# libshoal/Green-Marl

Measured on AMD Instinct MI355X. Metric: edges/s (GTEPS) per PageRank iter, RMAT-26, higher is better.
Workload: dtype f32; 1 GPU; pagerank RMAT-26 (V=67108864, E=1073741824), reference RMAT generator seed 1997 permute=1, d=0.85, fixed iterations; partition=1-D vertex, 1 rank(s), exchange=none, exchange_bytes_per_rank_and_step=0, exchange_packed=False, step_form=single rank, options=15

## Files before the change

### green-marl_amd/csrc/gmx_internal.h

```cpp
#ifndef GMX_INTERNAL_H_
#define GMX_INTERNAL_H_

#include <hip/hip_runtime.h>
#include <stdint.h>
#include <stdio.h>
#include <stdarg.h>
#include <string.h>
#include <time.h>
#include <stdlib.h>
#include <string>
#include <vector>

#include "gmx.h"

void gmx_set_error(const char* fmt, ...);

#define GMX_HIP(call)                                                                      \
    do {                                                                                   \
        hipError_t _e = (call);                                                            \
        if (_e != hipSuccess) {                                                            \
            gmx_set_error("%s:%d: %s -> %s", __FILE__, __LINE__, #call, hipGetErrorString(_e)); \
            return GMX_ERR_HIP;                                                            \
        }                                                                                  \
    } while (0)

#define GMX_CHECK(call)                 \
    do {                                \
        int _s = (call);                \
        if (_s != GMX_OK) return _s;    \
    } while (0)

#define GMX_REQUIRE(cond, ...)          \
    do {                                \
        if (!(cond)) {                  \
            gmx_set_error(__VA_ARGS__); \
            return GMX_ERR_ARG;         \
        }                               \
    } while (0)

template <typename T>
struct dbuf {
    T* p = nullptr;
    size_t n = 0;
    dbuf() {}
    dbuf(const dbuf&) = delete;
    dbuf& operator=(const dbuf&) = delete;
    ~dbuf() { release(); }
    int alloc(size_t count) {
        release();
        n = count;
        size_t bytes = (count ? count : 1) * sizeof(T);
        hipError_t e = hipMalloc((void**) &p, bytes);
        if (e != hipSuccess) {
            p = nullptr;
            n = 0;
            gmx_set_error("hipMalloc(%zu bytes) failed: %s", bytes, hipGetErrorString(e));
            return GMX_ERR_NOMEM;
        }
        return GMX_OK;
    }
    void release() {
        if (p) (void) hipFree(p);
        p = nullptr;
        n = 0;
    }
    T* take() { T* q = p; p = nullptr; n = 0; return q; }
};

struct gmx_event {
    hipEvent_t e = nullptr;
    gmx_event() {}
    gmx_event(gmx_event&& o) : e(o.e) { o.e = nullptr; }
    gmx_event(const gmx_event&) = delete;
    gmx_event& operator=(const gmx_event&) = delete;
    ~gmx_event() { if (e) (void) hipEventDestroy(e); }
    int create() { GMX_HIP(hipEventCreate(&e)); return GMX_OK; }
    operator hipEvent_t() const { return e; }
};
template <typename T>
struct gmx_pinned {
    T* p = nullptr;
    gmx_pinned() {}
    gmx_pinned(const gmx_pinned&) = delete;
    gmx_pinned& operator=(const gmx_pinned&) = delete;
    ~gmx_pinned() { if (p) (void) hipHostFree(p); }
    int alloc(size_t count = 1) {
        if (hipHostMalloc((void**) &p, count * sizeof(T), hipHostMallocDefault) != hipSuccess) {
            p = nullptr;
            gmx_set_error("pinned host allocation (%zu bytes) failed", count * sizeof(T));
            return GMX_ERR_HIP;
        }
        return GMX_OK;
    }
};
template <typename T>
static inline int gmx_read_back(gmx_pinned<T>& host, const T* dev, size_t count = 1) {
    GMX_HIP(hipMemcpyAsync(host.p, dev, count * sizeof(T), hipMemcpyDeviceToHost, 0));
    GMX_HIP(hipStreamSynchronize(0));
    return GMX_OK;
}

static inline int64_t gmx_env_int(const char* name, int64_t dflt, int64_t lo, int64_t hi) {
    const char* e = getenv(name);
    if (!e || !*e) return dflt;
    const long long v = atoll(e);
    return v < lo ? lo : (v > hi ? hi : (int64_t) v);
}

struct gmx_ws_mark { size_t chunk, off; };
void* gmx_ws_alloc(size_t bytes);
gmx_ws_mark gmx_ws_top();
void gmx_ws_rewind(gmx_ws_mark m);
struct gmx_ws_scope {
    gmx_ws_mark m;
    gmx_ws_scope() : m(gmx_ws_top()) {}
    ~gmx_ws_scope() { (void) hipDeviceSynchronize(); gmx_ws_rewind(m); }
    gmx_ws_scope(const gmx_ws_scope&) = delete;
    gmx_ws_scope& operator=(const gmx_ws_scope&) = delete;
};
template <typename T>
struct wbuf {
    T* p = nullptr;
    size_t n = 0;
    wbuf() {}
    wbuf(const wbuf&) = delete;
    wbuf& operator=(const wbuf&) = delete;
    int alloc(size_t count) {
        n = count;
        p = (T*) gmx_ws_alloc((count ? count : 1) * sizeof(T));
        if (!p) { n = 0; return GMX_ERR_NOMEM; }
        return GMX_OK;
    }
    void release() { p = nullptr; n = 0; }
};

struct gmx_bfs;
struct tcd_plan;
void gmx_tcd_plan_free(tcd_plan* p);
struct vc_plan;
void gmx_vc_plan_free(vc_plan* p);
struct spf_scratch;
void gmx_spf_scratch_free(spf_scratch* s);

struct gmx_graph {
    int64_t V = 0, E = 0;
    bool has_reverse = false;
    dbuf<int32_t> begin, node_idx, r_begin, r_node_idx;
    dbuf<int32_t> e_idx2idx;
    bool rows_sorted = true, r_rows_sorted = true;
    int device = 0;
    gmx_pr* pr_cache[4] = {nullptr, nullptr, nullptr, nullptr};
    struct gmx_pr_multi* pr_multi_cache[2] = {nullptr, nullptr};
    bool pr_multi_refused = false;
    int tc_sym_state = -1;
    gmx_graph* tc_oriented = nullptr;
    dbuf<uint32_t> tc_hub_bits;
    int64_t tc_hubs = 0;
    tcd_plan* tcd_cache = nullptr;
    vc_plan* vc_cache = nullptr;
    spf_scratch* spf_cache = nullptr;
    gmx_bfs* bfs_cache = nullptr;
    dbuf<int32_t> bfs_hint;
    dbuf<int32_t> bfs_hub_id;
    int64_t bfs_hubs = 0;
    bool bfs_hint_plain = false;
    gmx_graph* scc_transpose = nullptr;
};

int gmx_bfs_reach(gmx_graph* g, int32_t root, const int32_t** dist, int64_t* edges);
int gmx_bc_seeds(gmx_graph* g, const gmx_node_t* seeds, int32_t nseeds, int skip_root, float* bc_dev, bool zero_bc, hipEvent_t started, int64_t* reached);

int gmx_csr_from_keys(uint64_t* keys, uint64_t* keys_alt, int64_t V, int64_t E,
                      int32_t* begin, int32_t* idx, hipStream_t stream, int32_t* slots = nullptr);
int gmx_keys_from_csr(const int32_t* begin, const int32_t* idx, int64_t V, int64_t E,
                      bool transpose, const int32_t* perm, uint64_t* keys, hipStream_t stream);
int gmx_keys_from_edges(const int32_t* src, const int32_t* dst, int64_t E, bool transpose,
                        const int32_t* perm, uint64_t* keys, hipStream_t stream);
__global__ void iota_kernel(int32_t* __restrict__ a, int64_t n);

struct pr_cold;
struct pr_cold_params {
    int elem;
    int nranks;
    int64_t slice;
    int64_t T;
    int64_t row_lo;
    int64_t nactive;
    const int32_t* index_of_row;
    const int32_t* deg_by_id;
};
int pr_cold_create(const uint64_t* keys, int64_t Ec, const pr_cold_params& prm, hipStream_t s, pr_cold** out);
void pr_cold_free(pr_cold* c);
struct pr_cold_fuse {
    const int32_t* active;
    const int32_t* outdeg_c;
    void* rk_c;
    void* next_owned;
    double base, d;
};
int pr_cold_launch(pr_cold* c, const void* contrib, const pr_cold_fuse* fuse, hipStream_t s);
int pr_cold_set_parts(pr_cold* c, int nparts, const int64_t* act_bound, int64_t hub, int64_t live);
int pr_cold_parts(const pr_cold* c);
int64_t pr_cold_class_items(const pr_cold* c, int cls);
int pr_cold_gather(pr_cold* c, const void* contrib, int cls, hipStream_t s);
int pr_cold_accumulate(pr_cold* c, const pr_cold_fuse* fuse, int part, hipStream_t s);
const double* pr_cold_diff_partials(const pr_cold* c, int64_t* n);
bool pr_cold_covers_all_rows(const pr_cold* c);
bool pr_cold_limb_guard(const pr_cold* c, double d, double N);
const void* pr_cold_partial(const pr_cold* c);
int64_t pr_cold_edges(const pr_cold* c);
int64_t pr_cold_items(const pr_cold* c);

struct gmx_pr_multi;
int gmx_pr_multi_ranks(const gmx_graph* g);
int gmx_pr_multi_create(gmx_graph* g, int elem, int nranks, gmx_pr_multi** out);
int gmx_pr_multi_run(gmx_pr_multi* m, double e, double d, int32_t max_iter, void* rank_host, gmx_stats_t* stats);
void gmx_pr_multi_free(gmx_pr_multi* m);
bool gmx_pr_multi_verified(const gmx_pr_multi* m);

struct gmx_tick {
    bool on;
    double t0;
    const char* who;
    static double now() { struct timespec ts; clock_gettime(CLOCK_MONOTONIC, &ts); return ts.tv_sec + 1e-9 * ts.tv_nsec; }
    explicit gmx_tick(const char* w) : on(getenv("GMX_PLAN_TIMING") != nullptr), t0(0), who(w) { if (on) { (void) hipDeviceSynchronize(); t0 = now(); } }
    void mark(const char* what) {
        if (!on) return;
        (void) hipDeviceSynchronize();
        const double t = now();
        fprintf(stderr, "gmx timing %s: %-28s %8.2f ms\n", who, what, (t - t0) * 1e3);
        t0 = t;
    }
};

void gmx_touch_pagerank();
void gmx_touch_pr_cold();
void gmx_touch_bfs();
void gmx_touch_sssp();
void gmx_touch_nbrcount();
void gmx_touch_scc();
void gmx_touch_comm();
void gmx_touch_pf();
void gmx_touch_bc_batch();
void gmx_touch_tcd();
void gmx_touch_vcover();
void gmx_touch_match();
void gmx_touch_spf();
void gmx_touch_route();
void gmx_touch_walk();
void gmx_touch_wcc();
void gmx_touch_kcore();
void gmx_touch_msf();
void gmx_warm_modules();

static inline int gmx_bits_for(int64_t v) {
    int b = 1;
    while ((1LL << b) < v && b < 32) b++;
    return b;
}

#endif
```

### green-marl_amd/csrc/gmx_pr_cold.hip

```cpp
#pragma clang fp contract(off)

#include "gmx_internal.h"

#include <algorithm>
#include <rocprim/rocprim.hpp>

#define PRC_G 32
#define PRC_BLK_GROUPS 16
#define PRC_LDS_BYTES 131072
#define PRC_STAGE_BYTES 2048
#define PRC_LDS_LIMIT 163840
static constexpr int prc_tile_elems(int elem) { return (PRC_LDS_LIMIT - 16 * (PRC_STAGE_BYTES + 64 * elem) - 64) / elem; }
static constexpr int prc_tile_elems_classed(int elem) {
    return (PRC_LDS_LIMIT - 16 * 64 * elem - 64) / elem < 32768 ? (PRC_LDS_LIMIT - 16 * 64 * elem - 64) / elem / 8 * 8 : 32768;
}
#define PRC_THREADS 1024
#define PRC_WAVES (PRC_THREADS / 64)
#define PRC_UNROLL 4
#define PRC_PAD 0xffffu
#define PRC_END 0x8000u
#define PRC_Q1P 0
#define PRC_Q1E 64
#define PRC_Q2 128

// ... 564 lines not shown
#undef PRC_PROCESS
}

typedef float prc_f32x2 __attribute__((ext_vector_type(2)));
typedef double prc_f64x2 __attribute__((ext_vector_type(2)));

template <typename S, int FORM> struct prc_form_stores {
    static constexpr int NP = FORM == PRC_FORM_H ? 1 : 8 >> (FORM - PRC_FORM_E1);
    static constexpr int value = (NP * (int) sizeof(S) + 15) / 16;
};

template <typename S, int NP> __device__ __forceinline__ void prc_store_results(S* __restrict__ dst, const S (&out)[NP]);
template <> __device__ __forceinline__ void prc_store_results<float, 1>(float* __restrict__ dst, const float (&out)[1]) { __builtin_nontemporal_store(out[0], dst); }
template <> __device__ __forceinline__ void prc_store_results<float, 2>(float* __restrict__ dst, const float (&out)[2]) {
    prc_f32x2 v; v.x = out[0]; v.y = out[1];
    __builtin_nontemporal_store(v, (prc_f32x2*) dst);
}
template <> __device__ __forceinline__ void prc_store_results<float, 4>(float* __restrict__ dst, const float (&out)[4]) {
    prc_f32x4 v; v.x = out[0]; v.y = out[1]; v.z = out[2]; v.w = out[3];
    __builtin_nontemporal_store(v, (prc_f32x4*) dst);
}
template <> __device__ __forceinline__ void prc_store_results<float, 8>(float* __restrict__ dst, const float (&out)[8]) {
    prc_f32x4 a, b; a.x = out[0]; a.y = out[1]; a.z = out[2]; a.w = out[3]; b.x = out[4]; b.y = out[5]; b.z = out[6]; b.w = out[7];
    __builtin_nontemporal_store(a, (prc_f32x4*) dst);
    __builtin_nontemporal_store(b, (prc_f32x4*) dst + 1);
}
template <> __device__ __forceinline__ void prc_store_results<double, 1>(double* __restrict__ dst, const double (&out)[1]) { __builtin_nontemporal_store(out[0], dst); }
template <> __device__ __forceinline__ void prc_store_results<double, 2>(double* __restrict__ dst, const double (&out)[2]) {
    prc_f64x2 v; v.x = out[0]; v.y = out[1];
    __builtin_nontemporal_store(v, (prc_f64x2*) dst);
}
template <> __device__ __forceinline__ void prc_store_results<double, 4>(double* __restrict__ dst, const double (&out)[4]) {
#pragma unroll
    for (int q = 0; q < 2; q++) { prc_f64x2 v; v.x = out[2 * q]; v.y = out[2 * q + 1]; __builtin_nontemporal_store(v, (prc_f64x2*) dst + q); }
}
template <> __device__ __forceinline__ void prc_store_results<double, 8>(double* __restrict__ dst, const double (&out)[8]) {
#pragma unroll
    for (int q = 0; q < 4; q++) { prc_f64x2 v; v.x = out[2 * q]; v.y = out[2 * q + 1]; __builtin_nontemporal_store(v, (prc_f64x2*) dst + q); }
}

template <typename S, int L>
__device__ __forceinline__ void prc_block_E(const S* __restrict__ s_tile, const prc_u32x4 cur, const int32_t o, S* __restrict__ val, const int lane) {
    constexpr int NP = 8 / L;
    constexpr int K = (NP * (int) sizeof(S) + 15) / 16;
    const unsigned w[4] = {cur.x, cur.y, cur.z, cur.w};
    S fv[8];
#pragma unroll
    for (int u = 0; u < 8; u++) fv[u] = s_tile[__builtin_amdgcn_ubfe(w[u >> 1], 16 * (u & 1), 15)];
    S out[NP];
#pragma unroll
    for (int q = 0; q < NP; q++) {
        if (L == 1) out[q] = fv[q];
        else {
            double acc = (double) fv[q * L];
#pragma unroll
            for (int j = 1; j < L; j++) acc += (double) fv[q * L + j];
            out[q] = (S) acc;
        }
    }
    if constexpr (K == 1) {
        PRC_CHECK(o >= 0 && (o & (NP - 1)) == 0);
        prc_store_results<S, NP>(val + (o + (lane & 3) * NP), out);
    } else {
        constexpr int R = 16 / (int) sizeof(S), CPG = K / 2;
        const int o_lo = __builtin_amdgcn_update_dpp(0, o, 0x114, 0xf, 0xf, true);
        const int o_hi = __builtin_amdgcn_update_dpp(0, o, 0x104, 0xf, 0xf, true);
        const bool upper = (lane & 4) != 0;
        const int o_even = upper ? o_lo : o, o_odd = upper ? o : o_hi;
        const int m = lane & 7;
#pragma unroll
        for (int q = 0; q < K; q++) {
            S piece[R];
#pragma unroll
            for (int r = 0; r < R; r++) piece[r] = out[q * R + r];
            const int at = (q / CPG ? o_odd : o_even) + (q % CPG) * 8 * R + R * m;
            PRC_CHECK(at >= 0 && (at & (R - 1)) == 0);
            prc_store_results<S, R>(val + at, piece);
        }
    }
}

template <typename S>
__device__ __forceinline__ void prc_block_H(const S* __restrict__ s_tile, S* __restrict__ stage, const prc_u32x4 cur, const int32_t o,
                                            S* __restrict__ val, const unsigned sink, const int lane) {
    const unsigned w[4] = {cur.x, cur.y, cur.z, cur.w};
    S fv[8];
#pragma unroll
    for (int u = 0; u < 8; u++) fv[u] = s_tile[__builtin_amdgcn_ubfe(w[u >> 1], 16 * (u & 1), 15)];
    double v = (double) fv[0];
#pragma unroll
    for (int u = 1; u < 8; u++) v += (double) fv[u];
    const int endm = __builtin_amdgcn_sbfe((int) w[3], 31, 1);
    int f = prc_dpp_i<PRC_DPP_WAVE_SHR1, 0xf>(endm) & 1;
    prc_seg_step<PRC_DPP_ROW_SHR(1), 0xf>(v, f);
    prc_seg_step<PRC_DPP_ROW_SHR(2), 0xf>(v, f);
    prc_seg_step<PRC_DPP_ROW_SHR(4), 0xf>(v, f);
    prc_seg_step<PRC_DPP_ROW_SHR(8), 0xf>(v, f);
    prc_seg_step<PRC_DPP_BCAST15, 0xa>(v, f);
    prc_seg_step<PRC_DPP_BCAST31, 0xc>(v, f);
    const unsigned long long ends = __ballot(endm != 0);
    const int total = __builtin_popcountll(ends);
    const int ord = (int) __builtin_amdgcn_mbcnt_hi((unsigned) (ends >> 32), __builtin_amdgcn_mbcnt_lo((unsigned) ends, 0u));
    const unsigned g4 = (unsigned) (ends >> (lane & ~3)) & 0xfu;
    const int gbase = ord - __builtin_popcount(g4 & ((1u << (lane & 3)) - 1u));
    const int shift = o - gbase;
    const unsigned long long live = __ballot(g4 != 0u);
    const int shift0 = __builtin_amdgcn_readlane(shift, live ? __builtin_ctzll(live) : 0);
    const bool one_run = __ballot(g4 != 0u && shift != shift0) == 0ull;
    const S x = (S) v;
    unsigned at;
    S y;
    if (one_run) {
        if (endm) stage[ord] = x;
        __builtin_amdgcn_wave_barrier();
        __builtin_amdgcn_s_waitcnt(0xc07f);
        __builtin_amdgcn_wave_barrier();
        y = stage[lane];
        at = lane < total ? (unsigned) (shift0 + lane) : sink;
        __builtin_amdgcn_wave_barrier();
    } else {
        y = x;
        at = endm ? (unsigned) (shift + ord) : sink;
    }
    PRC_CHECK(at <= sink);
    val[at] = y;
}

template <typename S, int FORM>
__device__ __forceinline__ void prc_class_block(const S* __restrict__ s_tile, S* __restrict__ stage, const prc_u32x4 cur, const int32_t o,
                                                S* __restrict__ val, const unsigned sink, const int lane) {
    if constexpr (FORM == PRC_FORM_H) prc_block_H<S>(s_tile, stage, cur, o, val, sink, lane);
    else prc_block_E<S, 1 << (FORM - PRC_FORM_E1)>(s_tile, cur, o, val, lane);
}

#define PRC_SET_WAIT_N(t, N)                                                                                        \
    asm volatile("s_waitcnt vmcnt(%8)"                                                                              \
                 : "+v"((t).e0), "+v"((t).e1), "+v"((t).e2), "+v"((t).e3), "+v"((t).o0), "+v"((t).o1), "+v"((t).o2), "+v"((t).o3) \
                 : "n"(N) : "memory")

template <typename S, int FORM>
__device__ __forceinline__ void prc_class_item(const prc_item1 d, const S* __restrict__ s_tile, S* __restrict__ stage,
                                               const uint16_t* __restrict__ srcl, const int32_t* __restrict__ ob,
                                               S* __restrict__ val, const unsigned sink, const int wv, const int lane) {
    constexpr int NST = prc_form_stores<S, FORM>::value;
    const int nblocks = (d.g1 - d.g0) / PRC_BLK_GROUPS;
    const int nsuper = nblocks / (PRC_WAVES * PRC_PAIR_DEPTH);
    const prc_u32x4* in = (const prc_u32x4*) srcl + ((int64_t) d.g0 * (PRC_G / 8) + wv * 64 + lane);
    const int32_t* obp = ob + (d.g0 + wv * PRC_BLK_GROUPS + (lane >> 2));
    constexpr int64_t IN_STEP = PRC_PAIR_DEPTH * PRC_WAVES * 64;
    constexpr int64_t OB_STEP = PRC_PAIR_DEPTH * PRC_WAVES * PRC_BLK_GROUPS;
    if (nsuper > 0) {
        prc_set A, B;
#define PRC_PROCESS(t)                                                                  \
    do {                                                                                \
        prc_class_block<S, FORM>(s_tile, stage, (t).e0, (t).o0, val, sink, lane);       \
        prc_class_block<S, FORM>(s_tile, stage, (t).e1, (t).o1, val, sink, lane);       \
        prc_class_block<S, FORM>(s_tile, stage, (t).e2, (t).o2, val, sink, lane);       \
        prc_class_block<S, FORM>(s_tile, stage, (t).e3, (t).o3, val, sink, lane);       \
    } while (0)
        prc_set_load(A, in, obp);
        {
            const int kn = 1 < nsuper ? 1 : 0;
            prc_set_load(B, in + kn * IN_STEP, obp + kn * OB_STEP);
        }
        PRC_SET_WAIT_N(A, 8);
        PRC_PROCESS(A);
        int k = 1;
#pragma unroll 1
        for (; k + 1 < nsuper; k += 2) {
            prc_set_load(A, in + (int64_t) (k + 1) * IN_STEP, obp + (int64_t) (k + 1) * OB_STEP);
            PRC_SET_WAIT_N(B, 4 * NST + 8);
            PRC_PROCESS(B);
            const int kn = k + 2 < nsuper ? k + 2 : k + 1;
            prc_set_load(B, in + (int64_t) kn * IN_STEP, obp + (int64_t) kn * OB_STEP);
            PRC_SET_WAIT_N(A, 4 * NST + 8);
            PRC_PROCESS(A);
        }
        PRC_SET_WAIT_N(B, 4 * NST);
        if (k < nsuper) PRC_PROCESS(B);
#undef PRC_PROCESS
    }
    {
        const int b0 = nsuper * (PRC_WAVES * PRC_PAIR_DEPTH);
        prc_u32x4 cur[PRC_PAIR_DEPTH];
        int32_t o[PRC_PAIR_DEPTH];
#pragma unroll
        for (int j = 0; j < PRC_PAIR_DEPTH; j++)
            if (b0 + j * PRC_WAVES + wv < nblocks) {
                const int64_t off = (int64_t) (b0 + j * PRC_WAVES);
                cur[j] = __builtin_nontemporal_load(in + off * 64);
                o[j] = __builtin_nontemporal_load(obp + off * PRC_BLK_GROUPS);
            }
#pragma unroll
        for (int j = 0; j < PRC_PAIR_DEPTH; j++)
            if (b0 + j * PRC_WAVES + wv < nblocks) prc_class_block<S, FORM>(s_tile, stage, cur[j], o[j], val, sink, lane);
    }
}

template <typename S>
__device__ __forceinline__ void prc_edge_item(const prc_item1 d, const S* __restrict__ s_tile,
                                              const uint16_t* __restrict__ srcl, const int32_t* __restrict__ ob,
                                              S* __restrict__ val, const int wv, const int lane) {
    typedef typename prc_vec4<S>::type V4;
    const int npieces = (d.g1 - d.g0 + 7) >> 3;
    for (int base = 0; base < npieces; base += PRC_WAVES * PRC_UNROLL) {
        prc_u32x2 ids[PRC_UNROLL];
        int32_t o[PRC_UNROLL];
#pragma unroll
        for (int u = 0; u < PRC_UNROLL; u++) {
            const int pc = base + u * PRC_WAVES + wv;
            const int g = d.g0 + pc * 8 + (lane >> 3);
            o[u] = -1;
            if (pc < npieces && g < d.g1) {
                ids[u] = __builtin_nontemporal_load((const prc_u32x2*) srcl + (int64_t) g * (PRC_G / 4) + (lane & 7));
                o[u] = __builtin_nontemporal_load(ob + g);
            }
        }
#pragma unroll
        for (int u = 0; u < PRC_UNROLL; u++) {
            if (o[u] < 0) continue;
            V4 v;
            v.x = s_tile[ids[u].x & 0x7fffu];
            v.y = s_tile[(ids[u].x >> 16) & 0x7fffu];
            v.z = s_tile[ids[u].y & 0x7fffu];
            v.w = s_tile[(ids[u].y >> 16) & 0x7fffu];
            __builtin_nontemporal_store(v, (V4*) (val + o[u]) + (lane & 7));
        }
    }
}

template <typename S, int TILE, bool CLASSED>
__global__ void __launch_bounds__(PRC_THREADS)
pr_cold_tile_kernel(const prc_item1* __restrict__ items, int n_items, unsigned int* __restrict__ queue,
                    const S* __restrict__ contrib, const int32_t* __restrict__ org, int nranks, int64_t span, int64_t slice, int64_t T,
                    const uint16_t* __restrict__ srcl, const int32_t* __restrict__ ob, S* __restrict__ val, unsigned sink_base,
                    unsigned qbase, const int32_t* __restrict__ vst) {
    __shared__ S s_tile[TILE];
    __shared__ S s_stage[PRC_WAVES][CLASSED ? 64 : PRC_STAGE_BYTES / sizeof(S) + 64];
    __shared__ int s_item;
    const int tid = threadIdx.x, lane = tid & 63;
    const int wv = __builtin_amdgcn_readfirstlane(tid >> 6);
    const unsigned sink = sink_base + (blockIdx.x * PRC_WAVES + wv) * 64 + lane;
    int loaded = -1;
    for (;;) {
        __syncthreads();
        if (tid == 0) s_item = (int) (atomicAdd(&queue[CLASSED ? PRC_Q1E : PRC_Q1P], 1u) - qbase);
        __syncthreads();
        const int it = s_item;
        if ((unsigned) it >= (unsigned) n_items) break;
        const prc_item1 d = items[it];
        if (d.tile != loaded) {
            prc_load_tile<S, TILE>(s_tile, d.tile, org, contrib, nranks, span, slice, T);
            loaded = d.tile;
            __syncthreads();
        }
        if constexpr (CLASSED) {
            const int32_t* vs = vst + ((int64_t) d.tile << PRC_CLS_BITS);
            for (int cls = PRC_CL_E1; cls <= PRC_CL_H; cls++) {
                const int32_t lo = max(d.g0, vs[cls]), hi = min(d.g1, vs[cls + 1]);
                if (lo >= hi) continue;
                const prc_item1 seg{d.tile, lo, hi, cls + 1};
                switch (cls) {
                case PRC_CL_E1: prc_class_item<S, PRC_FORM_E1>(seg, s_tile, s_stage[wv], srcl, ob, val, sink, wv, lane); break;
                case PRC_CL_E2: prc_class_item<S, PRC_FORM_E2>(seg, s_tile, s_stage[wv], srcl, ob, val, sink, wv, lane); break;
                case PRC_CL_E4: prc_class_item<S, PRC_FORM_E4>(seg, s_tile, s_stage[wv], srcl, ob, val, sink, wv, lane); break;
                case PRC_CL_E8: prc_class_item<S, PRC_FORM_E8>(seg, s_tile, s_stage[wv], srcl, ob, val, sink, wv, lane); break;
                default: prc_class_item<S, PRC_FORM_H>(seg, s_tile, s_stage[wv], srcl, ob, val, sink, wv, lane); break;
                }
            }
        } else {
            if (d.form == PRC_FORM_PAIR) prc_pair_item<S>(d, s_tile, s_stage[wv], srcl, ob, val, sink, wv, lane);
            else prc_edge_item<S>(d, s_tile, srcl, ob, val, wv, lane);
        }
    }
}

__device__ __forceinline__ unsigned long long prc_fix_hi(double v) { return (unsigned long long) (long long) (v * 0x1p62); }

template <typename S>
__device__ __forceinline__ void prc_finish_row(const pr_cold_fuse& fz, int64_t i, double sum, double& diff_acc) {
    const int32_t od = __builtin_nontemporal_load(fz.outdeg_c + i);
    const int64_t r = __builtin_nontemporal_load(fz.active + i);
    const double old = (double) __builtin_nontemporal_load((const S*) fz.rk_c + i);
    const S vs = (S) (fz.base + fz.d * sum);
    diff_acc += fabs((double) vs - old);
    __builtin_nontemporal_store(vs, (S*) fz.rk_c + i);
    __builtin_nontemporal_store(od > 0 ? (S) ((double) vs / (double) od) : (S) 0, (S*) fz.next_owned + r);
}

template <int THREADS>
__device__ __forceinline__ void prc_block_diff(double diff_acc, double* s_red, double* __restrict__ dst) {
#pragma unroll
    for (int off = 32; off > 0; off >>= 1) diff_acc += __shfl_down(diff_acc, off, 64);
    if ((threadIdx.x & 63) == 0) s_red[threadIdx.x >> 6] = diff_acc;
    __syncthreads();
    if (threadIdx.x == 0) {
        double t = 0.0;
#pragma unroll
        for (int w = 0; w < THREADS / 64; w++) t += s_red[w];
        *dst = t;
    }
}

template <typename S, int BINROWS, int LIMBS, bool FUSE>
__global__ void __launch_bounds__(PRC_THREADS)
pr_cold_accum_kernel(const prc_item2* __restrict__ items, int n_items, unsigned int* __restrict__ queue,
                     const uint16_t* __restrict__ rowl, const S* __restrict__ val, int64_t nactive, double lo_scale,
                     S* __restrict__ cold, unsigned long long* __restrict__ scratch, pr_cold_fuse fz,
                     double* __restrict__ diff_part, unsigned qbase) {
    typedef typename prc_vec4<S>::type V4;
    __shared__ unsigned long long s_acc[LIMBS * BINROWS];
    __shared__ double s_red[PRC_WAVES];
    __shared__ int s_item;
    const int tid = threadIdx.x, lane = tid & 63;
    const int wv = __builtin_amdgcn_readfirstlane(tid >> 6);
    for (;;) {
        __syncthreads();
        if (tid == 0) s_item = (int) (atomicAdd(&queue[PRC_Q2], 1u) - qbase);
#pragma unroll 4
        for (int i = tid; i < LIMBS * BINROWS; i += PRC_THREADS) s_acc[i] = 0ull;
        __syncthreads();
        const int it = s_item;
        if ((unsigned) it >= (unsigned) n_items) break;
        const prc_item2 d = items[it];
        const int npieces = (d.g1 - d.g0 + 7) >> 3;
        for (int base = 0; base < npieces; base += PRC_WAVES * PRC_UNROLL) {
            prc_u32x2 ids[PRC_UNROLL];
            V4 v[PRC_UNROLL];
            bool ok[PRC_UNROLL];
#pragma unroll
            for (int u = 0; u < PRC_UNROLL; u++) {
                const int pc = base + u * PRC_WAVES + wv;
                const int g = d.g0 + pc * 8 + (lane >> 3);
                ok[u] = pc < npieces && g < d.g1;
                if (ok[u]) {
                    const int64_t at = (int64_t) g * (PRC_G / 4) + (lane & 7);
                    ids[u] = __builtin_nontemporal_load((const prc_u32x2*) rowl + at);
                    v[u] = __builtin_nontemporal_load((const V4*) val + at);
                }
            }
#pragma unroll
            for (int u = 0; u < PRC_UNROLL; u++) {
                if (!ok[u]) continue;
                const unsigned r[4] = {ids[u].x & 0xffffu, ids[u].x >> 16, ids[u].y & 0xffffu, ids[u].y >> 16};
                const double x[4] = {(double) v[u].x, (double) v[u].y, (double) v[u].z, (double) v[u].w};
#pragma unroll
                for (int j = 0; j < 4; j++) {
                    if (r[j] == PRC_PAD) continue;
                    PRC_CHECK(r[j] < (unsigned) BINROWS && x[j] >= 0.0 && x[j] <= 1.0);
                    const unsigned long long hi = prc_fix_hi(x[j]);
                    __hip_atomic_fetch_add(&s_acc[r[j]], hi, __ATOMIC_RELAXED, __HIP_MEMORY_SCOPE_WORKGROUP);
                    if (LIMBS > 1) {
                        const double rem = x[j] - (double) (long long) hi * 0x1p-62;
                        const unsigned long long lo = (unsigned long long) (long long) (rem * 0x1p62 * lo_scale);
                        __hip_atomic_fetch_add(&s_acc[BINROWS + r[j]], lo, __ATOMIC_RELAXED, __HIP_MEMORY_SCOPE_WORKGROUP);
                    }
                }
            }
        }
        __syncthreads();
        double diff_acc = 0.0;
        if (d.slot < 0) {
            const int64_t i0 = (int64_t) d.bin * BINROWS;
#pragma unroll 4
            for (int r = tid; r < BINROWS; r += PRC_THREADS) {
                if (i0 + r >= nactive) break;
                double sum = (double) (long long) s_acc[r] * 0x1p-62;
                if (LIMBS > 1) sum += (double) (long long) s_acc[BINROWS + r] * (0x1p-62 / lo_scale);
                if (FUSE) prc_finish_row<S>(fz, i0 + r, sum, diff_acc);
                else __builtin_nontemporal_store((S) sum, cold + i0 + r);
            }
        } else {
            unsigned long long* dst = scratch + (int64_t) d.slot * (LIMBS * BINROWS);
#pragma unroll 4
            for (int i = tid; i < LIMBS * BINROWS; i += PRC_THREADS) dst[i] = s_acc[i];
        }
        if (FUSE) prc_block_diff<PRC_THREADS>(diff_acc, s_red, diff_part + it);
    }
}

template <typename S, int BINROWS, int LIMBS, bool FUSE>
__global__ void __launch_bounds__(1024)
pr_cold_reduce_kernel(const prc_item3* __restrict__ items, int64_t nactive, double lo_scale,
                      const unsigned long long* __restrict__ scratch, S* __restrict__ cold, pr_cold_fuse fz,
                      double* __restrict__ diff_part) {
    __shared__ unsigned long long s_part[LIMBS][16][64];
    const prc_item3 d = items[blockIdx.y];
    const int lane = threadIdx.x & 63, wv = threadIdx.x >> 6;
    const int r = blockIdx.x * 64 + lane;
    const int64_t i0 = (int64_t) d.bin * BINROWS;
    unsigned long long hi = 0, lo = 0;
    const unsigned long long* src = scratch + (int64_t) d.slot0 * (LIMBS * BINROWS) + r;
#pragma unroll 4
    for (int s = wv; s < d.nslots; s += 16) {
        hi += __builtin_nontemporal_load(src + (int64_t) s * (LIMBS * BINROWS));
        if (LIMBS > 1) lo += __builtin_nontemporal_load(src + (int64_t) s * (LIMBS * BINROWS) + BINROWS);
    }
    s_part[0][wv][lane] = hi;
    if (LIMBS > 1) s_part[LIMBS - 1][wv][lane] = lo;
    __syncthreads();
    if (wv == 0 && i0 + r < nactive) {
        hi = 0;
        lo = 0;
#pragma unroll
        for (int w = 0; w < 16; w++) {
            hi += s_part[0][w][lane];
            if (LIMBS > 1) lo += s_part[LIMBS - 1][w][lane];
        }
        double v = (double) (long long) hi * 0x1p-62;
        if (LIMBS > 1) v += (double) (long long) lo * (0x1p-62 / lo_scale);
        if (FUSE) {
            double diff_acc = 0.0;
            prc_finish_row<S>(fz, i0 + r, v, diff_acc);
            s_part[0][0][lane] = (unsigned long long) __double_as_longlong(diff_acc);
        } else cold[i0 + r] = (S) v;
    } else if (FUSE && wv == 0) s_part[0][0][lane] = 0ull;
    if (FUSE && wv == 0) {
        __builtin_amdgcn_wave_barrier();
        __builtin_amdgcn_s_waitcnt(0xc07f);
        __builtin_amdgcn_wave_barrier();
        if (lane == 0) {
            double t = 0.0;
            for (int l = 0; l < 64; l++) t += __longlong_as_double((long long) s_part[0][0][l]);
            diff_part[(int64_t) blockIdx.y * gridDim.x + blockIdx.x] = t;
        }
    }
}

#define PRC_FEW_SLOTS 8
template <typename S, int BINROWS, int LIMBS, bool FUSE>
__global__ void __launch_bounds__(256)
pr_cold_reduce_few_kernel(const prc_item3* __restrict__ items, int64_t nactive, double lo_scale,
                          const unsigned long long* __restrict__ scratch, S* __restrict__ cold, pr_cold_fuse fz,
                          double* __restrict__ diff_part) {
    const prc_item3 d = items[blockIdx.y];
    const int lane = threadIdx.x & 63;
    const int rg = blockIdx.x * 4 + (threadIdx.x >> 6);
    const int r = rg * 64 + lane;
    const int64_t i0 = (int64_t) d.bin * BINROWS;
    unsigned long long hi = 0, lo = 0;
    const unsigned long long* src = scratch + (int64_t) d.slot0 * (LIMBS * BINROWS) + r;
#pragma unroll 4
    for (int s = 0; s < d.nslots; s++) {
        hi += __builtin_nontemporal_load(src + (int64_t) s * (LIMBS * BINROWS));
        if (LIMBS > 1) lo += __builtin_nontemporal_load(src + (int64_t) s * (LIMBS * BINROWS) + BINROWS);
    }
    double diff_acc = 0.0;
    if (i0 + r < nactive) {
        double v = (double) (long long) hi * 0x1p-62;
        if (LIMBS > 1) v += (double) (long long) lo * (0x1p-62 / lo_scale);
        if (FUSE) prc_finish_row<S>(fz, i0 + r, v, diff_acc);
        else cold[i0 + r] = (S) v;
    }
    if (FUSE) {
        double t = 0.0;
        for (int l = 0; l < 64; l++) t += __shfl(diff_acc, l, 64);
        if (lane == 0) diff_part[(int64_t) blockIdx.y * (BINROWS / 64) + rg] = t;
    }
}

static int prc_upload_lists(pr_cold* c, const std::vector<uint8_t>* tile_class, const std::vector<int32_t>* bin_part, int nparts) {
    auto by_size1 = [](const prc_item1& a, const prc_item1& b) { return a.g1 - a.g0 > b.g1 - b.g0; };
    auto by_size2 = [](const prc_item2& a, const prc_item2& b) { return a.g1 - a.g0 > b.g1 - b.g0; };
    std::vector<prc_item1> l1;
    for (int k = 0; k < 2; k++) {
        c->o1[k] = (int64_t) l1.size();
        for (int part = 0; part < 3; part++) {
            if (part == 1) c->o1g[k] = (int64_t) l1.size();
            std::vector<prc_item1> a;
            for (const prc_item1& it : (part < 2 ? c->h1p : c->h1e))
                if ((tile_class ? (int) (*tile_class)[(size_t) it.tile] : 0) == k && (part == 2 || (part == 0) == (it.form >= PRC_FORM_E1))) a.push_back(it);
            std::stable_sort(a.begin(), a.end(), by_size1);
            l1.insert(l1.end(), a.begin(), a.end());
        }
    }
    c->o1[2] = (int64_t) l1.size();
    std::vector<prc_item2> l2;
    std::vector<prc_item3> l3;
    c->o2.assign((size_t) nparts + 1, 0);
    c->o3.assign((size_t) nparts + 1, 0);
    c->o3few.assign((size_t) nparts, 0);
    for (int q = 0; q < nparts; q++) {
        c->o2[(size_t) q] = (int64_t) l2.size();
        c->o3[(size_t) q] = (int64_t) l3.size();
        std::vector<prc_item2> a;
        for (const prc_item2& it : c->h2)
            if ((bin_part ? (*bin_part)[(size_t) it.bin] : 0) == q) a.push_back(it);
        std::stable_sort(a.begin(), a.end(), by_size2);
        l2.insert(l2.end(), a.begin(), a.end());
        for (int few = 1; few >= 0; few--)
            for (const prc_item3& it : c->h3)
                if ((bin_part ? (*bin_part)[(size_t) it.bin] : 0) == q && (it.nslots <= PRC_FEW_SLOTS ? 1 : 0) == few) {
                    l3.push_back(it);
                    if (few) c->o3few[(size_t) q]++;
                }
    }
    c->o2[(size_t) nparts] = (int64_t) l2.size();
    c->o3[(size_t) nparts] = (int64_t) l3.size();
    c->nparts = nparts;
    if ((int64_t) l1.size() != c->n1p + c->n1e || (int64_t) l2.size() != c->n2 || (int64_t) l3.size() != c->n3) {
        gmx_set_error("pr cold: work lists lost items while being regrouped");
        return GMX_ERR_ARG;
    }
    if (!l1.empty()) GMX_HIP(hipMemcpy(c->it1p.p, l1.data(), sizeof(prc_item1) * l1.size(), hipMemcpyHostToDevice));
    if (!l2.empty()) GMX_HIP(hipMemcpy(c->it2.p, l2.data(), sizeof(prc_item2) * l2.size(), hipMemcpyHostToDevice));
    if (!l3.empty()) GMX_HIP(hipMemcpy(c->it3.p, l3.data(), sizeof(prc_item3) * l3.size(), hipMemcpyHostToDevice));
    return GMX_OK;
}

int pr_cold_set_parts(pr_cold* c, int nparts, const int64_t* act_bound, int64_t hub, int64_t live) {
    if (!c || c->Ec == 0) return GMX_OK;
    if (nparts <= 1) return prc_upload_lists(c, nullptr, nullptr, 1);
    std::vector<int32_t> bin_part((size_t) c->nbins, 0);
    {
        std::vector<int64_t> bb((size_t) nparts + 1, 0);
        for (int j = 1; j < nparts; j++) bb[(size_t) j] = std::min<int64_t>(c->nbins, act_bound[j] / c->binrows);
        bb[(size_t) nparts] = c->nbins;
        for (int j = 0; j < nparts; j++)
            for (int64_t b = bb[(size_t) j]; b < bb[(size_t) j + 1]; b++) bin_part[(size_t) b] = nparts - 1 - j;
    }
    std::vector<uint8_t> tile_class((size_t) c->ntiles, 0);
    const int64_t span = c->prm.slice - c->prm.T, tile_src = c->tile - 1;
    for (int64_t t = 0; t < c->ntiles; t++) {
        const int64_t cp0 = t * tile_src, cp1 = std::min<int64_t>(cp0 + tile_src, span * c->prm.nranks);
        bool hub_only = true;
        for (int64_t r = cp0 / span; r * span < cp1 && hub_only; r++) {
            const int64_t o0 = c->prm.T + std::max<int64_t>(cp0, r * span) - r * span;
            const int64_t o1 = c->prm.T + std::min<int64_t>(cp1, (r + 1) * span) - r * span;
            if (o0 < live && std::min(o1, live) > hub) hub_only = false;
        }
        tile_class[(size_t) t] = hub_only ? 0 : 1;
    }
    return prc_upload_lists(c, &tile_class, &bin_part, nparts);
}

int pr_cold_parts(const pr_cold* c) { return c ? c->nparts : 1; }
int64_t pr_cold_class_items(const pr_cold* c, int cls) { return c && cls >= 0 && cls < 2 ? c->o1[cls + 1] - c->o1[cls] : 0; }

#define PRC_TRY(expr, what)                                                                  \
    do {                                                                                     \
        hipError_t _e = (expr);                                                              \
        if (_e != hipSuccess) {                                                              \
            gmx_set_error("pr cold plan: %s failed: %s", what, hipGetErrorString(_e));       \
            st = GMX_ERR_HIP;                                                                \
            goto done;                                                                       \
        }                                                                                    \
    } while (0)
#define PRC_ALLOC(buf, count)                        \
    do {                                             \
        if ((st = (buf).alloc((size_t) (count)))) goto done; \
    } while (0)

static int prc_env_int(const char* name, int dflt) {
    const char* v = getenv(name);
    return v && *v ? atoi(v) : dflt;
}

static hipError_t prc_exscan(const int32_t* in, int32_t* out, int64_t n, wbuf<char>& tmp, hipStream_t s) {
    size_t tb = 0;
    hipError_t e = rocprim::exclusive_scan(nullptr, tb, in, out, 0, (size_t) n, rocprim::plus<int32_t>(), s);
    if (e != hipSuccess) return e;
    if (tmp.n < tb) {
        tmp.release();
        if (tmp.alloc(tb)) return hipErrorOutOfMemory;
    }
    return rocprim::exclusive_scan((void*) tmp.p, tb, in, out, 0, (size_t) n, rocprim::plus<int32_t>(), s);
}

static hipError_t prc_inscan(const int32_t* in, int32_t* out, int64_t n, wbuf<char>& tmp, hipStream_t s) {
    size_t tb = 0;
    hipError_t e = rocprim::inclusive_scan(nullptr, tb, in, out, (size_t) n, rocprim::plus<int32_t>(), s);
    if (e != hipSuccess) return e;
    if (tmp.n < tb) {
        tmp.release();
        if (tmp.alloc(tb)) return hipErrorOutOfMemory;
    }
    return rocprim::inclusive_scan((void*) tmp.p, tb, in, out, (size_t) n, rocprim::plus<int32_t>(), s);
}

int pr_cold_create(const uint64_t* keys, int64_t Ec, const pr_cold_params& prm, hipStream_t s, pr_cold** outp) {
    *outp = nullptr;
    GMX_REQUIRE(prm.elem == 4 || prm.elem == 8, "pr cold: bad element size");
    GMX_REQUIRE(prm.T >= 0 && prm.T < prm.slice, "pr cold: threshold outside the rank range");
    GMX_REQUIRE(Ec < (1LL << 31) - (1LL << 27), "pr cold: %lld edges exceed the int32 stream positions", (long long) Ec);
    pr_cold* c = new pr_cold();
    c->prm = prm;
    c->Ec = Ec;
    const int64_t class_density = prc_env_int("GMX_PR_COLD_CLASS_DENSITY", 1);
    const bool all_classed = class_density == 1;
    c->tile = all_classed ? prc_tile_elems_classed(prm.elem) : prc_tile_elems(prm.elem);
    const int tile_src = c->tile - 1;
    c->limbs = prm.elem == 4 ? 1 : 2;
    c->binrows = PRC_LDS_BYTES / 8 / c->limbs;
    c->ncold = (int64_t) prm.nranks * (prm.slice - prm.T);
    c->ntiles = (c->ncold + tile_src - 1) / tile_src;
    c->nbins = (prm.nactive + c->binrows - 1) / c->binrows;
    if (c->nbins < 1) c->nbins = 1;
    const int tilebits = gmx_bits_for(c->ntiles), binbits = gmx_bits_for(c->nbins), vtbits = tilebits + PRC_CLS_BITS;
    const int64_t nvt = c->ntiles << PRC_CLS_BITS;
    const double pair_min = prc_env_int("GMX_PR_COLD_PAIR_X100", 125) / 100.0;
    int st = GMX_OK;
    gmx_tick tick("cold plan");
    gmx_ws_scope ws;
    wbuf<uint64_t> k1, k2;
    wbuf<int32_t> cflag, cincl, ps, pincl, pstart, plen, ppos, pos, endf, endpre, first, pfirst, groups, c1raw, c1, vtab, delta, counts, id, order2, groups2,
        c2s, c2, tab2, tstat;
    wbuf<uint32_t> ckey, key2, key2s;
    wbuf<uint8_t> mode;
    wbuf<char> tmp;
    uint64_t* sk = nullptr;
    std::vector<int32_t> hts, hvt, hdelta, vstart, h2;
    std::vector<uint8_t> hmode;
    std::vector<prc_item1> v1p, v1e;
    std::vector<prc_item2> v2;
    std::vector<prc_item3> v3;
    int64_t ngroups1 = 0, ngroups2 = 0, nc = 0, np = 0, pair_edges = 0, pair_tiles = 0, class_tiles = 0, class_edges = 0;
    hipDeviceProp_t prop;
    int dev = 0;
    if (vtbits + binbits > 32) {
        gmx_set_error("pr cold: %lld tiles x %lld bins do not fit the sort key", (long long) c->ntiles, (long long) c->nbins);
        st = GMX_ERR_ARG;
        goto done;
    }
    PRC_ALLOC(c->cold, (size_t) (prm.nactive ? prm.nactive : 1) * prm.elem);
    PRC_TRY(hipMemsetAsync(c->cold.p, 0, (size_t) (prm.nactive ? prm.nactive : 1) * prm.elem, s), "memset");
    PRC_ALLOC(c->queue, 3 * 64);
    PRC_TRY(hipMemsetAsync(c->queue.p, 0, 3 * 64 * sizeof(unsigned int), s), "memset");
    (void) hipGetDevice(&dev);
    PRC_TRY(hipGetDeviceProperties(&prop, dev), "hipGetDeviceProperties");
    c->grid = prop.multiProcessorCount;
    if (Ec == 0) {
        PRC_TRY(hipStreamSynchronize(s), "sync");
        *outp = c;
        return GMX_OK;
    }
    {
        PRC_ALLOC(k1, Ec);
        PRC_ALLOC(k2, Ec);
        hipLaunchKernelGGL(prc_keys_kernel, dim3(prc_grid_for(Ec)), dim3(256), 0, s, keys, Ec, prm, tile_src, c->binrows, binbits, k1.p);
        rocprim::double_buffer<uint64_t> db(k1.p, k2.p);
        size_t tb = 0;
        const unsigned end_bit = 32u + (unsigned) binbits + (unsigned) vtbits;
        PRC_TRY(rocprim::radix_sort_keys(nullptr, tb, db, (size_t) Ec, 16u, end_bit, s), "sort size");
        PRC_ALLOC(tmp, tb);
        PRC_TRY(rocprim::radix_sort_keys((void*) tmp.p, tb, db, (size_t) Ec, 16u, end_bit, s), "sort");
        PRC_TRY(hipStreamSynchronize(s), "sort sync");
        sk = db.current();
    }
    tick.mark("keys + main sort");
    PRC_ALLOC(cflag, Ec + 1);
    PRC_ALLOC(cincl, Ec + 1);
    PRC_ALLOC(ps, Ec + 1);
    PRC_ALLOC(pincl, Ec + 1);
    PRC_ALLOC(mode, c->ntiles + 1);
    PRC_ALLOC(tstat, 3 * (c->ntiles + 1));
    hmode.assign((size_t) c->ntiles + 1, PRC_TM_EDGE);
    for (int round = 0; round < 2; round++) {
        hipLaunchKernelGGL(prc_runs_kernel, dim3(prc_grid_for(Ec)), dim3(256), 0, s, (const uint64_t*) sk, Ec,
                           round ? (const uint8_t*) mode.p : (const uint8_t*) nullptr, 32 + binbits + PRC_CLS_BITS, cflag.p, ps.p);
        PRC_TRY(prc_inscan(cflag.p, cincl.p, Ec, tmp, s), "scan");
        PRC_TRY(prc_inscan(ps.p, pincl.p, Ec, tmp, s), "scan");
        {
            int32_t lastc = 0, lastp = 0;
            PRC_TRY(hipMemcpyAsync(&lastc, cincl.p + (Ec - 1), 4, hipMemcpyDeviceToHost, s), "copy");
            PRC_TRY(hipMemcpyAsync(&lastp, pincl.p + (Ec - 1), 4, hipMemcpyDeviceToHost, s), "copy");
            PRC_TRY(hipStreamSynchronize(s), "sync");
            c->ncells = nc = lastc;
            np = lastp;
        }
        if (pstart.n < (size_t) np + 1) { pstart.release(); PRC_ALLOC(pstart, np + 1); }
        hipLaunchKernelGGL(prc_pair_start_kernel, dim3(prc_grid_for(Ec + 1)), dim3(256), 0, s, (const int32_t*) ps.p, (const int32_t*) pincl.p, Ec, np, pstart.p);
        if (round == 1) break;
        hipLaunchKernelGGL(prc_tile_stats_kernel, dim3(prc_grid_for(c->ntiles + 1)), dim3(256), 0, s, (const uint64_t*) sk, Ec,
                           32 + binbits + PRC_CLS_BITS, c->ntiles, (const int32_t*) pincl.p, (const int32_t*) cincl.p, np, nc, tstat.p);
        hts.resize((size_t) 3 * (c->ntiles + 1));
        PRC_TRY(hipMemcpyAsync(hts.data(), tstat.p, sizeof(int32_t) * hts.size(), hipMemcpyDeviceToHost, s), "copy");
        PRC_TRY(hipStreamSynchronize(s), "sync");
        for (int64_t t = 0; t < c->ntiles; t++) {
// ... 369 lines not shown
```

Measured before the change: 800.1 GTEPS.

## Double-buffer cold accumulate loads, branch-free f32 fixed-point atomics, batched fused finish

The cold accumulate kernel now loads edge batches with ping-pong register buffers, so the next batch's global loads are in flight while the current batch's LDS atomics run. Padded and out-of-range lanes no longer branch. They are sent to per-lane dump slots appended to the LDS accumulator, and for f32 with one limb the fixed-point conversion uses an integer bit-shift instead of double arithmetic. The fused finish issues all of a thread's row loads (outdeg, active, old rank) up front and waits once before computing. The cost is more registers and LDS, which may lower occupancy, and the asm wait pin forces a full vmcnt drain.

```diff
diff --git a/green-marl_amd/csrc/gmx_internal.h b/green-marl_amd/csrc/gmx_internal.h
--- a/green-marl_amd/csrc/gmx_internal.h
+++ b/green-marl_amd/csrc/gmx_internal.h
@@ -191,6 +191,12 @@
 };
 int pr_cold_create(const uint64_t* keys, int64_t Ec, const pr_cold_params& prm, hipStream_t s, pr_cold** out);
 void pr_cold_free(pr_cold* c);
+__host__ __device__ static inline unsigned long long gmx_prc_fix_f32(uint32_t bits) {
+    const uint32_t e = (bits >> 23) & 0xffu, m = (bits & 0x7fffffu) | 0x800000u;
+    const uint32_t k = 127u - e;
+    return ((unsigned long long) m << 39) >> (k < 63u ? k : 63u);
+}
+
 struct pr_cold_fuse {
     const int32_t* active;
     const int32_t* outdeg_c;
diff --git a/green-marl_amd/csrc/gmx_pr_cold.hip b/green-marl_amd/csrc/gmx_pr_cold.hip
--- a/green-marl_amd/csrc/gmx_pr_cold.hip
+++ b/green-marl_amd/csrc/gmx_pr_cold.hip
@@ -890,78 +890,158 @@
     }
 }
 
+#define PRC_ACC_STRIDE(binrows) ((binrows) + PRC_THREADS)
+template <typename S> struct prc_batch {
+    prc_u32x2 ids[PRC_UNROLL];
+    typename prc_vec4<S>::type v[PRC_UNROLL];
+};
+template <typename S>
+__device__ __forceinline__ void prc_batch_load(prc_batch<S>& b, const uint16_t* __restrict__ rowl, const S* __restrict__ val,
+                                               const prc_item2 d, const int batch, const int wv, const int lane) {
+    typedef typename prc_vec4<S>::type V4;
+#pragma unroll
+    for (int u = 0; u < PRC_UNROLL; u++) {
+        const int g = d.g0 + ((batch * PRC_UNROLL + u) * PRC_WAVES + wv) * 8 + (lane >> 3);
+        const int64_t at = (int64_t) min(g, d.g1 - 1) * (PRC_G / 4) + (lane & 7);
+        b.ids[u] = __builtin_nontemporal_load((const prc_u32x2*) rowl + at);
+        b.v[u] = __builtin_nontemporal_load((const V4*) val + at);
+    }
+}
+template <typename S, int BINROWS, int LIMBS>
+__device__ __forceinline__ void prc_batch_add(const prc_batch<S>& b, unsigned long long* __restrict__ s_acc, const prc_item2 d,
+                                              const int batch, const int wv, const int lane, const double lo_scale) {
+    const unsigned dump = BINROWS + wv * 64 + lane;
+#pragma unroll
+    for (int u = 0; u < PRC_UNROLL; u++) {
+        const int g = d.g0 + ((batch * PRC_UNROLL + u) * PRC_WAVES + wv) * 8 + (lane >> 3);
+        const bool past = g >= d.g1;
+        const unsigned w0 = past ? 0xffffffffu : b.ids[u].x, w1 = past ? 0xffffffffu : b.ids[u].y;
+        const unsigned r[4] = {w0 & 0xffffu, w0 >> 16, w1 & 0xffffu, w1 >> 16};
+        const S xs[4] = {b.v[u].x, b.v[u].y, b.v[u].z, b.v[u].w};
+#pragma unroll
+        for (int j = 0; j < 4; j++) {
+            const bool live = r[j] != PRC_PAD;
+            PRC_CHECK(!live || r[j] < (unsigned) BINROWS);
+            if constexpr (sizeof(S) == 4 && LIMBS == 1) {
+                const unsigned at = live ? r[j] : dump;
+                const uint32_t bits = live ? __float_as_uint((float) xs[j]) : 0u;
+                PRC_CHECK(bits <= 0x3f800000u || bits == 0x80000000u);
+                __hip_atomic_fetch_add(&s_acc[at], gmx_prc_fix_f32(bits), __ATOMIC_RELAXED, __HIP_MEMORY_SCOPE_WORKGROUP);
+            } else if (live) {
+                const double x = (double) xs[j];
+                PRC_CHECK(x >= 0.0 && x <= 1.0);
+                const unsigned long long hi = prc_fix_hi(x);
+                __hip_atomic_fetch_add(&s_acc[r[j]], hi, __ATOMIC_RELAXED, __HIP_MEMORY_SCOPE_WORKGROUP);
+                if (LIMBS > 1) {
+                    const double rem = x - (double) (long long) hi * 0x1p-62;
+                    const unsigned long long lo = (unsigned long long) (long long) (rem * 0x1p62 * lo_scale);
+                    __hip_atomic_fetch_add(&s_acc[PRC_ACC_STRIDE(BINROWS) + r[j]], lo, __ATOMIC_RELAXED, __HIP_MEMORY_SCOPE_WORKGROUP);
+                }
+            }
+        }
+    }
+}
+
+template <typename S>
+__device__ __forceinline__ void prc_pin8(const int32_t* od, const int32_t* act, const S* old) {
+    asm volatile("s_waitcnt vmcnt(0)"
+                 :: "v"(od[0]), "v"(od[1]), "v"(od[2]), "v"(od[3]), "v"(od[4]), "v"(od[5]), "v"(od[6]), "v"(od[7]),
+                    "v"(act[0]), "v"(act[1]), "v"(act[2]), "v"(act[3]), "v"(act[4]), "v"(act[5]), "v"(act[6]), "v"(act[7]),
+                    "v"(old[0]), "v"(old[1]), "v"(old[2]), "v"(old[3]), "v"(old[4]), "v"(old[5]), "v"(old[6]), "v"(old[7]));
+}
+template <typename S, int BINROWS, int LIMBS, int ROWS>
+__device__ __forceinline__ void prc_finish_rows(const pr_cold_fuse& fz, const unsigned long long* __restrict__ s_acc,
+                                                const int64_t i0, const int r0, const int64_t nactive, const double lo_scale,
+                                                double& diff_acc) {
+    int32_t od[ROWS], act[ROWS];
+    S old[ROWS];
+#pragma unroll
+    for (int k = 0; k < ROWS; k++) {
+        const int64_t i = min(i0 + r0 + k * PRC_THREADS, nactive - 1);
+        od[k] = __builtin_nontemporal_load(fz.outdeg_c + i);
+        act[k] = __builtin_nontemporal_load(fz.active + i);
+        old[k] = __builtin_nontemporal_load((const S*) fz.rk_c + i);
+    }
+#pragma unroll
+    for (int k = 0; k < ROWS; k += 8) prc_pin8<S>(od + k, act + k, old + k);
+#pragma unroll
+    for (int k = 0; k < ROWS; k++) {
+        const int r = r0 + k * PRC_THREADS;
+        double sum = (double) (long long) s_acc[r] * 0x1p-62;
+        if (LIMBS > 1) sum += (double) (long long) s_acc[PRC_ACC_STRIDE(BINROWS) + r] * (0x1p-62 / lo_scale);
+        const S vs = (S) (fz.base + fz.d * sum);
+        if (i0 + r < nactive) {
+            diff_acc += fabs((double) vs - (double) old[k]);
+            __builtin_nontemporal_store(vs, (S*) fz.rk_c + i0 + r);
+            __builtin_nontemporal_store(od[k] > 0 ? (S) ((double) vs / (double) od[k]) : (S) 0, (S*) fz.next_owned + (int64_t) act[k]);
+        }
+    }
+}
+
 template <typename S, int BINROWS, int LIMBS, bool FUSE>
 __global__ void __launch_bounds__(PRC_THREADS)
 pr_cold_accum_kernel(const prc_item2* __restrict__ items, int n_items, unsigned int* __restrict__ queue,
                      const uint16_t* __restrict__ rowl, const S* __restrict__ val, int64_t nactive, double lo_scale,
                      S* __restrict__ cold, unsigned long long* __restrict__ scratch, pr_cold_fuse fz,
                      double* __restrict__ diff_part, unsigned qbase) {
-    typedef typename prc_vec4<S>::type V4;
-    __shared__ unsigned long long s_acc[LIMBS * BINROWS];
+    constexpr int STRIDE = PRC_ACC_STRIDE(BINROWS);
+    __shared__ unsigned long long s_acc[LIMBS * STRIDE];
     __shared__ double s_red[PRC_WAVES];
     __shared__ int s_item;
+    static_assert(sizeof(unsigned long long) * LIMBS * STRIDE + sizeof(double) * PRC_WAVES + sizeof(int) <= PRC_LDS_LIMIT, "LDS of a CU");
     const int tid = threadIdx.x, lane = tid & 63;
     const int wv = __builtin_amdgcn_readfirstlane(tid >> 6);
     for (;;) {
         __syncthreads();
         if (tid == 0) s_item = (int) (atomicAdd(&queue[PRC_Q2], 1u) - qbase);
+#pragma unroll
+        for (int l = 0; l < LIMBS; l++)
 #pragma unroll 4
-        for (int i = tid; i < LIMBS * BINROWS; i += PRC_THREADS) s_acc[i] = 0ull;
+            for (int i = tid; i < BINROWS; i += PRC_THREADS) s_acc[l * STRIDE + i] = 0ull;
         __syncthreads();
         const int it = s_item;
         if ((unsigned) it >= (unsigned) n_items) break;
         const prc_item2 d = items[it];
-        const int npieces = (d.g1 - d.g0 + 7) >> 3;
-        for (int base = 0; base < npieces; base += PRC_WAVES * PRC_UNROLL) {
-            prc_u32x2 ids[PRC_UNROLL];
-            V4 v[PRC_UNROLL];
-            bool ok[PRC_UNROLL];
-#pragma unroll
-            for (int u = 0; u < PRC_UNROLL; u++) {
-                const int pc = base + u * PRC_WAVES + wv;
-                const int g = d.g0 + pc * 8 + (lane >> 3);
-                ok[u] = pc < npieces && g < d.g1;
-                if (ok[u]) {
-                    const int64_t at = (int64_t) g * (PRC_G / 4) + (lane & 7);
-                    ids[u] = __builtin_nontemporal_load((const prc_u32x2*) rowl + at);
-                    v[u] = __builtin_nontemporal_load((const V4*) val + at);
-                }
+        const int nbatches = (d.g1 - d.g0 + 8 * PRC_WAVES * PRC_UNROLL - 1) / (8 * PRC_WAVES * PRC_UNROLL);
+        if (nbatches > 0) {
+            prc_batch<S> A, B;
+            prc_batch_load<S>(A, rowl, val, d, 0, wv, lane);
+            int k = 1;
+#pragma unroll 1
+            for (; k + 1 < nbatches; k += 2) {
+                prc_batch_load<S>(B, rowl, val, d, k, wv, lane);
+                prc_batch_add<S, BINROWS, LIMBS>(A, s_acc, d, k - 1, wv, lane, lo_scale);
+                prc_batch_load<S>(A, rowl, val, d, k + 1, wv, lane);
+                prc_batch_add<S, BINROWS, LIMBS>(B, s_acc, d, k, wv, lane, lo_scale);
             }
-#pragma unroll
-            for (int u = 0; u < PRC_UNROLL; u++) {
-                if (!ok[u]) continue;
-                const unsigned r[4] = {ids[u].x & 0xffffu, ids[u].x >> 16, ids[u].y & 0xffffu, ids[u].y >> 16};
-                const double x[4] = {(double) v[u].x, (double) v[u].y, (double) v[u].z, (double) v[u].w};
-#pragma unroll
-                for (int j = 0; j < 4; j++) {
-                    if (r[j] == PRC_PAD) continue;
-                    PRC_CHECK(r[j] < (unsigned) BINROWS && x[j] >= 0.0 && x[j] <= 1.0);
-                    const unsigned long long hi = prc_fix_hi(x[j]);
-                    __hip_atomic_fetch_add(&s_acc[r[j]], hi, __ATOMIC_RELAXED, __HIP_MEMORY_SCOPE_WORKGROUP);
-                    if (LIMBS > 1) {
-                        const double rem = x[j] - (double) (long long) hi * 0x1p-62;
-                        const unsigned long long lo = (unsigned long long) (long long) (rem * 0x1p62 * lo_scale);
-                        __hip_atomic_fetch_add(&s_acc[BINROWS + r[j]], lo, __ATOMIC_RELAXED, __HIP_MEMORY_SCOPE_WORKGROUP);
-                    }
-                }
-            }
+            const bool one_more = k < nbatches;
+            if (one_more) prc_batch_load<S>(B, rowl, val, d, k, wv, lane);
+            prc_batch_add<S, BINROWS, LIMBS>(A, s_acc, d, k - 1, wv, lane, lo_scale);
+            if (one_more) prc_batch_add<S, BINROWS, LIMBS>(B, s_acc, d, k, wv, lane, lo_scale);
         }
         __syncthreads();
         double diff_acc = 0.0;
         if (d.slot < 0) {
             const int64_t i0 = (int64_t) d.bin * BINROWS;
+            if (FUSE) {
+                constexpr int ROWS = BINROWS / PRC_THREADS;
+                static_assert(ROWS == 8 || ROWS == 16, "the finish keeps the three loads of all of a thread's rows in registers");
+                if (i0 < nactive) prc_finish_rows<S, BINROWS, LIMBS, ROWS>(fz, s_acc, i0, tid, nactive, lo_scale, diff_acc);
+            } else {
 #pragma unroll 4
-            for (int r = tid; r < BINROWS; r += PRC_THREADS) {
-                if (i0 + r >= nactive) break;
-                double sum = (double) (long long) s_acc[r] * 0x1p-62;
-                if (LIMBS > 1) sum += (double) (long long) s_acc[BINROWS + r] * (0x1p-62 / lo_scale);
-                if (FUSE) prc_finish_row<S>(fz, i0 + r, sum, diff_acc);
-                else __builtin_nontemporal_store((S) sum, cold + i0 + r);
+                for (int r = tid; r < BINROWS; r += PRC_THREADS) {
+                    if (i0 + r >= nactive) break;
+                    double sum = (double) (long long) s_acc[r] * 0x1p-62;
+                    if (LIMBS > 1) sum += (double) (long long) s_acc[STRIDE + r] * (0x1p-62 / lo_scale);
+                    __builtin_nontemporal_store((S) sum, cold + i0 + r);
+                }
             }
         } else {
             unsigned long long* dst = scratch + (int64_t) d.slot * (LIMBS * BINROWS);
+#pragma unroll
+            for (int l = 0; l < LIMBS; l++)
 #pragma unroll 4
-            for (int i = tid; i < LIMBS * BINROWS; i += PRC_THREADS) dst[i] = s_acc[i];
+                for (int i = tid; i < BINROWS; i += PRC_THREADS) dst[l * BINROWS + i] = s_acc[l * STRIDE + i];
         }
         if (FUSE) prc_block_diff<PRC_THREADS>(diff_acc, s_red, diff_part + it);
     }
```

Result: slower. 788.5 GTEPS (-1.5%).
